# bcgsc/NanoSim

Measured on NVIDIA H100. Metric: simulated_bases_per_sec, higher is better.
Workload: dtype u8

## Files before the change

nanosim_b200/csrc/emit_kernel.cuh:

```cuda
#pragma once
#include "device_common.cuh"

#define EMIT_WARPS 8
#define EMIT_RING 256
#ifndef EMIT_MIN_BLOCKS
#define EMIT_MIN_BLOCKS 3
#endif

#ifndef EMIT_TMA_WINDOW
#define EMIT_TMA_WINDOW 1
#endif
#define EMIT_WIN_WORDS 64
#define EMIT_WINDOW_SMEM (EMIT_TMA_WINDOW ? EMIT_WARPS * (EMIT_WIN_WORDS * 4 + 8) : 0)

#define EMIT_F_RND 1u
#define EMIT_F_REF 4u
#define EMIT_F_MIS 8u

struct EmitArgs {
    DevRef ref;
    DevCfg cfg;
    uint32_t kind;
    uint32_t force_exact;
    uint64_t first_id;
    const NsReadMeta* reads;
    const NsPieceMeta* pieces;
    const uint32_t* ops;
    uint32_t n_pieces;
    uint8_t* seq;
    uint8_t* qual;
    const uint32_t* qlut;
    uint32_t* counter;
    const uint32_t* order;
    const uint32_t* abort;
    const uint32_t* split_base;
    const uint2* extra;
    const uint4* ckpt;
    const uint32_t* n_extra;
    uint32_t cap_extra;
};

#define EMIT_SPLIT 16384u

__device__ __forceinline__ uint32_t warp_incl_scan(uint32_t v, int lane) {
#pragma unroll
    for (int d = 1; d < 32; d <<= 1) {
        uint32_t t = __shfl_up_sync(0xffffffffu, v, d);
        if (lane >= d) v += t;
    }
    return v;
}

__device__ __forceinline__ uint32_t emit_op_info(uint32_t op, bool unmapped, bool ref_comp = false) {
    const uint32_t ty = op >> 28;
    const uint32_t qs = unmapped ? 4u : (ty == NS_OP_LIT ? ((op >> 24) & 3u) : ((0x30102u >> (4u * ty)) & 7u));
    uint32_t info = (qs * QLUT_SIZE * 4u) << 16;
    const uint32_t zero = ref_comp ? (uint32_t)'T' : (uint32_t)'A';
    if (ty < 2u) info |= EMIT_F_REF | (ty == NS_OP_MIS ? EMIT_F_MIS : 0u) | (zero << 8);
    else if (ty == NS_OP_LIT) info |= idx_base(((op >> 26) & 3u) ^ (ref_comp ? 2u : 0u)) << 8;
    else info |= 3u | (zero << 8);
    return info;
}

struct ChunkAux {
    uint32_t RB;
    uint32_t X[3];
};
template <bool FASTQ>
struct ChunkQual {
    uint32_t W[FASTQ ? 16 : 1];
    uint32_t X[4];
};

template <bool FASTQ>
__device__ __forceinline__ void draw_chunk_aux(ChunkAux& r, uint32_t id_lo, uint32_t id_hi, uint32_t kind, uint32_t chunk, uint2 key) {
    const uint4 a = FASTQ ? philox4x32_7(make_uint4(id_lo, id_hi, stream_word(ST_EMIT_Q, kind, chunk), 4u), key)
                          : philox4x32_7(make_uint4(id_lo, id_hi, stream_word(ST_EMIT_B, kind, chunk), 0u), key);
    r.RB = a.x; r.X[0] = a.y; r.X[1] = a.z; r.X[2] = a.w;
}
template <bool FASTQ>
__device__ __forceinline__ void draw_chunk_qual(ChunkQual<FASTQ>& r, uint32_t id_lo, uint32_t id_hi, uint32_t kind, uint32_t chunk, uint2 key) {
    if (FASTQ) {
        const uint32_t sw = stream_word(ST_EMIT_Q, kind, chunk);
#pragma unroll
        for (int j = 0; j < 4; ++j) {
            const uint4 t = philox4x32_7(make_uint4(id_lo, id_hi, sw, (uint32_t)j), key);
            r.W[4 * j] = t.x; r.W[4 * j + 1] = t.y; r.W[4 * j + 2] = t.z; r.W[4 * j + 3] = t.w;
            r.X[j] = __byte_perm(__byte_perm(t.x, t.y, 0x0040), __byte_perm(t.z, t.w, 0x0040), 0x5410);
        }
    } else {
        const uint4 b = philox4x32_7(make_uint4(id_lo, id_hi, stream_word(ST_EMIT_B, kind, chunk), 1u), key);
        r.X[0] = b.x; r.X[1] = b.y; r.X[2] = b.z; r.X[3] = b.w;
        r.W[0] = 0;
    }
}

__device__ __forceinline__ uint32_t sub_offsets(const uint32_t (&XA)[3], const uint32_t (&XB)[4]) {
    uint32_t sub = XA[0];
#pragma unroll
    for (int j = 1; j < 7; ++j) {
        const uint32_t z = ~(sub | (sub >> 1)) & 0x55555555u;
        sub |= (j < 3 ? XA[j] : XB[j - 3]) & (z * 3u);
    }
    return sub | (~(sub | (sub >> 1)) & 0x55555555u);
}
__device__ __forceinline__ uint32_t add_fields_mod4(uint32_t a, uint32_t b) {
    return a ^ b ^ ((a & b & 0x55555555u) << 1);
}

__device__ __forceinline__ uint32_t qual_pick(uint32_t e, uint32_t w) {
    return ((w | 0x7ffffu) < e) ? e : (e >> 8);
}

struct EmitPiece {
    const uint8_t* cbase;
    uint32_t pos, clen;
    uint32_t rdir;
    uint32_t ref_comp;
    uint32_t tbl;
    uint32_t piece_in_read;
    uint64_t rid;
};

__device__ __forceinline__ uint32_t entry_ref(const uint4& e, uint32_t rdir, uint32_t p) { return rdir ? e.y - p : e.y + p; }

__device__ __noinline__ uint32_t emit_fix_base(const EmitArgs& a, const EmitPiece& pc, const uint4* ring, uint32_t w_ret,
                                               uint32_t w_loaded, uint32_t x, uint32_t rb2, uint32_t misoff) {
    uint32_t l = w_ret, h = w_loaded;
    while (h - l > 1) {
        uint32_t mid = (l + h) >> 1;
        if (ring[mid & (EMIT_RING - 1)].x <= 2u * x) l = mid; else h = mid;
    }
    const uint4 e = ring[l & (EMIT_RING - 1)];
    const uint32_t info = e.w;
    uint32_t oi;
    if (info & EMIT_F_REF) {
        uint32_t rabs = entry_ref(e, pc.rdir, x);
        if (rabs >= pc.clen) rabs += pc.rdir ? pc.clen : 0u - pc.clen;
        uint32_t c = __ldg(pc.cbase + rabs);
        if (c - 'a' < 26u) c -= 32;
        if (!acgt_fast(c)) {
            const uint32_t f = rabs >= pc.pos ? rabs - pc.pos : rabs + pc.clen - pc.pos;
            c = converted_ref_base(c, a.cfg.seed, pc.rid, pc.piece_in_read, f);
        }
        oi = base_idx(c) ^ (pc.ref_comp ? 2u : 0u);
        if (info & EMIT_F_MIS) oi = (oi + misoff) & 3u;
    } else {
        oi = (info & 3u) ? rb2 : (base_idx((info >> 8) & 0xffu) ^ (pc.ref_comp ? 2u : 0u));
    }
    return (pc.tbl >> (8u * oi)) & 0xffu;
}

template <bool FASTQ, bool WRAPS, bool COMP>
__device__ __forceinline__ void emit_chunk16(const uint4* ring, const uint32_t* lut, const uint8_t* cvt_tables,
                                             const uint8_t* __restrict__ cbase, uint32_t RB, uint32_t sub, const ChunkQual<FASTQ>& Q,
                                             uint32_t& k, uint32_t& rem, uint32_t& rabs, uint32_t& info, uint32_t rdir, uint32_t clen,
                                             uint32_t wrap_fix, uint32_t tbl, uint32_t (&sb)[4], uint32_t (&sq)[4], uint32_t& bad) {
    const uint8_t* cvt = cvt_tables + (COMP ? 256 : 0);
    const uint32_t dir = rdir ? 0xffffffffu : 1u;
    uint32_t sel = 0;
#pragma unroll
    for (int i = 0; i < 16; ++i) {
        if (rem == 0) {
            ++k;
            const uint4 e = ring[k & (EMIT_RING - 1)];
            rem = (e.z - e.x) >> 1;
            rabs = entry_ref(e, rdir, e.x >> 1);
            info = e.w;
        }
        --rem;
        uint32_t c = (info >> 8) & 0xffu;
        if (info & EMIT_F_REF) {
            c = __ldg(cbase + rabs);
            rabs += dir;
            if (WRAPS && rabs >= clen) rabs += wrap_fix;
        }
        const uint32_t code = cvt[c];
        bad |= code;
        uint32_t v = code | ((RB >> (2 * i)) & info & 3u);
        if (info & EMIT_F_MIS) v += (sub >> (2 * i)) & 3u;
        sel += v << (4 * (i & 3));
        if (FASTQ) {
            const uint32_t w = Q.W[i];
            const uint32_t e = *reinterpret_cast<const uint32_t*>(reinterpret_cast<const char*>(lut) + (info >> 16) +
                                                                  ((w >> 6) & 0x1ffcu));
            sq[i >> 2] |= (qual_pick(e, w) & 0xffu) << (8 * (i & 3));
        }
        if ((i & 3) == 3) {
            sb[i >> 2] = __byte_perm(tbl, 0, sel & 0x3333u);
            sel = 0;
        }
    }
}

__device__ __forceinline__ uint32_t reverse_pairs(uint32_t x) {
    x = __brev(x);
    return ((x & 0x55555555u) << 1) | ((x >> 1) & 0x55555555u);
}
__device__ __forceinline__ uint32_t spread_pairs(uint32_t h) {
    uint32_t t = (h | (h << 8)) & 0x00ff00ffu;
    t = (t | (t << 4)) & 0x0f0f0f0fu;
    return (t | (t << 2)) & 0x33333333u;
}
__device__ __forceinline__ uint32_t bit_mask(uint32_t pos, uint32_t width) {
    uint32_t m;
    asm("bmsk.clamp.b32 %0, %1, %2;" : "=r"(m) : "r"(pos), "r"(width));
    return m;
}

__device__ __forceinline__ void load_packed_pair(const uint32_t* __restrict__ pk, uint32_t widx, uint32_t win_s, uint32_t win_w0,
                                                 uint32_t& w0, uint32_t& w1) {
#if EMIT_TMA_WINDOW
    const uint32_t rel = widx - win_w0;
    if (rel < EMIT_WIN_WORDS - 1u) {
        asm("ld.shared.u32 %0, [%2];\n\tld.shared.u32 %1, [%2+4];" : "=r"(w0), "=r"(w1) : "r"(win_s + 4u * rel));
        return;
    }
#endif
    w0 = __ldg(pk + widx);
    w1 = __ldg(pk + widx + 1);
}

template <bool RDIR>
__device__ __forceinline__ uint32_t emit_walk_entries(uint32_t ring_s, const uint32_t* __restrict__ pk, uint32_t pk0w, uint32_t win_s,
                                                      uint32_t win_w0, uint32_t RB, uint32_t& k, uint32_t cs, uint32_t& S, uint32_t& mism) {
    uint32_t acc = 0;
    S = 0xaaaaaaaau;
    mism = 0;
    const uint32_t cs2 = 2u * cs;
    for (;;) {
        uint4 e;
        asm("ld.shared.v4.u32 {%0, %1, %2, %3}, [%4];" : "=r"(e.x), "=r"(e.y), "=r"(e.z), "=r"(e.w) : "r"(ring_s + ((k & (EMIT_RING - 1)) << 4)));
        const uint32_t info = e.w;
        const int32_t d0 = (int32_t)(e.x - cs2);
        const uint32_t lo2 = (uint32_t)(d0 > 0 ? d0 : 0);
        const uint32_t d1 = e.z - cs2;
        const uint32_t hi2 = d1 < 32u ? d1 : 32u;
        const uint32_t m = bit_mask(lo2, hi2 - lo2);
        if (info & EMIT_F_REF) {
            const uint32_t p = cs + (lo2 >> 1);
            uint32_t r16;
            if (!RDIR) {
                const uint32_t l = e.y + p;
                uint32_t w0, w1;
                load_packed_pair(pk, pk0w + (l >> 4), win_s, win_w0, w0, w1);
                r16 = __funnelshift_r(w0, w1, (l + l) & 30u);
            } else {
                const uint32_t l1 = e.y - p + 1u;
                uint32_t w0, w1;
                load_packed_pair(pk, pk0w + (l1 >> 4) - 1u, win_s, win_w0, w0, w1);
                r16 = reverse_pairs(__funnelshift_r(w0, w1, (l1 + l1) & 30u));
            }
            acc = (acc & ~m) | ((r16 << lo2) & m);
            if (info & EMIT_F_MIS) mism |= m;
        } else {
            const uint32_t v = (info & EMIT_F_RND) ? RB : ((info >> 9) & 3u) * 0x55555555u;
            acc = (acc & ~m) | (v & m);
            S = (S & ~m) | (((info >> 29) * 0x55555555u) & m);
        }
        if (d1 >= 32u) break;
        ++k;
    }
    return acc;
}

template <bool FASTQ>
__device__ __forceinline__ void emit_chunk16_fast(uint32_t ring_s, const char* lut_s, const uint32_t* __restrict__ pk, uint32_t pk0w,
                                                  uint32_t win_s, uint32_t win_w0, uint32_t& k,
                                                  uint32_t cs, bool rdir, bool unmapped, uint32_t tbl, uint32_t id_lo, uint32_t id_hi,
                                                  uint32_t kind, uint32_t chunk, uint2 key, uint32_t (&sb)[4], uint32_t (&sq)[4]) {
    ChunkAux R;
    draw_chunk_aux<FASTQ>(R, id_lo, id_hi, kind, chunk, key);
    uint32_t S, mism;
    uint32_t acc = rdir ? emit_walk_entries<true>(ring_s, pk, pk0w, win_s, win_w0, R.RB, k, cs, S, mism)
                        : emit_walk_entries<false>(ring_s, pk, pk0w, win_s, win_w0, R.RB, k, cs, S, mism);
    ChunkQual<FASTQ> Q;
    draw_chunk_qual<FASTQ>(Q, id_lo, id_hi, kind, chunk, key);
    acc = add_fields_mod4(acc, sub_offsets(R.X, Q.X) & mism);
    S &= ~mism;
    {
        const uint32_t s0 = spread_pairs(acc & 0xffffu), s1 = spread_pairs(acc >> 16);
        sb[0] = __byte_perm(tbl, 0, s0);
        sb[1] = __byte_perm(tbl, 0, s0 >> 16);
        sb[2] = __byte_perm(tbl, 0, s1);
        sb[3] = __byte_perm(tbl, 0, s1 >> 16);
    }
    if (FASTQ) {
        if (unmapped) S = 0;
        uint32_t q[16];
#pragma unroll
        for (int i = 0; i < 16; ++i) {
            const uint32_t w = Q.W[i];
            const uint32_t st = (2 * i <= 13) ? (S << (13 - 2 * i)) : (S >> (2 * i - 13));
            const uint32_t off = (st & 0x6000u) | ((w >> 6) & 0x1ffcu);
            q[i] = qual_pick(*reinterpret_cast<const uint32_t*>(lut_s + off), w);
        }
#pragma unroll
        for (int g = 0; g < 4; ++g)
            sq[g] = __byte_perm(__byte_perm(q[4 * g], q[4 * g + 1], 0x0040), __byte_perm(q[4 * g + 2], q[4 * g + 3], 0x0040), 0x5410);
    }
}

template <bool FASTQ>
__global__ void __launch_bounds__(EMIT_WARPS * 32, EMIT_MIN_BLOCKS) emit_kernel(const __grid_constant__ EmitArgs a) {
    if (a.abort && *a.abort) return;
    extern __shared__ uint4 smem4[];
    uint32_t* lut = reinterpret_cast<uint32_t*>(smem4);
    uint8_t* cvt_tables = reinterpret_cast<uint8_t*>(lut + (FASTQ ? NS_N_QUAL_STATES * QLUT_SIZE : 0));
    const int lane = threadIdx.x & 31, warp = threadIdx.x >> 5;
    uint4* ring = reinterpret_cast<uint4*>(cvt_tables + 512) + warp * EMIT_RING;
    const uint32_t ring_s = (uint32_t)__cvta_generic_to_shared(ring);
#if EMIT_TMA_WINDOW
    const uint32_t win_s = (uint32_t)__cvta_generic_to_shared(reinterpret_cast<uint4*>(cvt_tables + 512) + EMIT_WARPS * EMIT_RING) +
                           warp * (EMIT_WIN_WORDS * 4);
    const uint32_t mbar_s = win_s + (EMIT_WARPS - warp) * (EMIT_WIN_WORDS * 4) + warp * 8;
    uint32_t win_phase = 0;
    if (lane == 0) {
        asm volatile("mbarrier.init.shared::cta.b64 [%0], 1;" ::"r"(mbar_s));
        asm volatile("fence.mbarrier_init.release.cluster;" ::: "memory");
    }
#else
    const uint32_t win_s = 0;
#endif
    if (FASTQ)
        for (int i = threadIdx.x; i < NS_N_QUAL_STATES * QLUT_SIZE; i += blockDim.x) lut[i] = a.qlut[i];
    {
        uint32_t c = threadIdx.x;
        uint32_t u = (c - 'a' < 26u) ? c - 32u : c;
        cvt_tables[c] = (uint8_t)(acgt_fast(u) ? base_idx(u) : 4u);
        cvt_tables[256 + c] = (uint8_t)(acgt_fast(u) ? base_idx(u) ^ 2u : 4u);
    }
    __syncthreads();
    const uint2 key = make_uint2((uint32_t)a.cfg.seed, (uint32_t)(a.cfg.seed >> 32));
    const uint32_t lane_lt = (1u << lane) - 1u;

    uint32_t n_extra = a.split_base ? *a.n_extra : 0u;
    if (n_extra > a.cap_extra) n_extra = a.cap_extra;
    for (;;) {
        uint32_t piece = 0, sub = 0;
        if (lane == 0) piece = atomicAdd(a.counter, 1u);
        piece = __shfl_sync(0xffffffffu, piece, 0);
        if (piece >= n_extra + a.n_pieces) break;
        if (piece < n_extra) {
            const uint2 x = a.extra[piece];
            if (x.x == 0xffffffffu) continue;
            piece = x.x;
            sub = x.y;
        } else {
            piece -= n_extra;
            if (a.order) piece = __ldg(&a.order[piece]);
        }
        const NsPieceMeta pm = a.pieces[piece];
        if (pm.out_len == 0) continue;
        const NsReadMeta rm = a.reads[pm.read_slot];
        const bool rev = rm.reversed != 0;
        const bool ref_comp = (pm.kind & NS_PIECE_REF_REV) != 0;
        const bool rdir = rev != ref_comp;
        const uint32_t n_ops = pm.n_ops, ref_len = pm.ref_len;
        const uint32_t A = rev ? rm.seq_len - pm.out_rel - pm.out_len : pm.out_rel;
        uint32_t pad = A & 15u;
        const uint32_t P0 = A - pad;
        uint32_t x_end = pad + pm.out_len;
        uint32_t t_first = 0, out_first = pad, ref_first = 0, x_first = 0;
        {
            const uint32_t sbase = a.split_base ? __ldg(&a.split_base[piece]) : 0xffffffffu;
            if (sbase != 0xffffffffu) {
                if (sub) {
                    const uint4 ck = a.ckpt[sbase + sub - 1u];
                    t_first = ck.x;
                    out_first = ck.y;
                    ref_first = ck.z;
                    x_first = sub * EMIT_SPLIT;
                    pad = 0;
                }
                if (x_end > (sub + 1u) * EMIT_SPLIT) x_end = (sub + 1u) * EMIT_SPLIT;
            }
        }
        const uint64_t cstart = a.ref.chrom_off[pm.chrom];
        EmitPiece pc;
        pc.cbase = a.ref.bases + cstart;
        pc.pos = pm.pos;
        pc.clen = (uint32_t)(a.ref.chrom_off[pm.chrom + 1] - cstart);
        pc.rdir = rdir;
        pc.ref_comp = ref_comp;
        {
            const uint32_t t = a.cfg.uracil ? 0x47554341u : 0x47544341u;
            pc.tbl = rev ? __byte_perm(t, 0, 0x1032) : t;
        }
        pc.piece_in_read = piece - rm.piece_first;
        pc.rid = a.first_id + pm.read_slot;
        const uint8_t* __restrict__ cbase = pc.cbase;
        const uint32_t clen = pc.clen, tbl = pc.tbl;
        const bool wraps = (uint64_t)pm.pos + ref_len > clen;
        const uint32_t wrap_fix = rdir ? clen : 0u - clen;
        const uint32_t* __restrict__ ops = a.ops + pm.op_off;
        uint8_t* seq_out = a.seq + rm.seq_off + P0;
        uint8_t* qual_out = FASTQ ? a.qual + rm.seq_off + P0 : nullptr;
        const bool unmapped = NS_PIECE_KIND(pm.kind) != NS_PIECE_SEGMENT;
        const uint32_t id_lo = (uint32_t)pc.rid, id_hi = (uint32_t)(pc.rid >> 32);
        const uint32_t info_pad = emit_op_info(NS_OP_HT << 28, unmapped, ref_comp);
        const uint64_t pk0 = a.ref.pk_off[pm.chrom];
        bool fast = !wraps && !ref_comp && !a.force_exact;
        if (fast && ref_len) {
            const uint64_t w_lo = pk0 + (pm.pos >> 4), w_hi = pk0 + ((pm.pos + ref_len - 1u) >> 4);
            fast = __ldg(&a.ref.exc_pre[(w_hi >> REF_EXC_BLOCK_SHIFT) + 1]) == __ldg(&a.ref.exc_pre[w_lo >> REF_EXC_BLOCK_SHIFT]);
        }
        const char* lut_s = reinterpret_cast<const char*>(lut) + (unmapped ? 4u * QLUT_SIZE * 4u : 0u);

        uint32_t t_loaded = t_first, w_loaded = 0, w_ret = 0, out_loaded = out_first, ref_loaded = ref_first, prog = x_first;
        bool closed = false;
        if (pad) {
            if (lane == 0) ring[0] = make_uint4(0u, 0u, 2u * pad, info_pad);
            w_loaded = 1;
        }
        auto put_entry = [&](uint32_t slot, uint32_t xo, uint32_t rstart, uint32_t len, uint32_t op) {
            uint32_t ab = pm.pos + (rdir ? ref_len - 1u - rstart : rstart);
            if (wraps && ab >= clen) ab -= clen;
            ring[slot & (EMIT_RING - 1)] = make_uint4(2u * xo, rdir ? ab + xo : ab - xo, 2u * (xo + len), emit_op_info(op, unmapped, ref_comp));
        };
        while (prog < x_end) {
            uint32_t target = prog + 512u < x_end ? prog + 512u : x_end;
            while (out_loaded < target && t_loaded < n_ops && (w_loaded - w_ret) + 65u <= EMIT_RING) {
                const uint32_t t = t_loaded + 2u * lane;
                uint32_t op0 = 0, op1 = 0;
                if (t < n_ops) op0 = __ldg(&ops[rev ? n_ops - 1u - t : t]);
                if (t + 1u < n_ops) op1 = __ldg(&ops[rev ? n_ops - 2u - t : t + 1u]);
                const uint32_t ty0 = op0 >> 28, len0 = op_len(op0), ty1 = op1 >> 28, len1 = op_len(op1);
                const uint32_t o0 = (ty0 == NS_OP_DEL) ? 0u : len0, o1 = (ty1 == NS_OP_DEL) ? 0u : len1;
                const uint32_t r0 = (ty0 < 2u || ty0 == NS_OP_DEL) ? len0 : 0u, r1 = (ty1 < 2u || ty1 == NS_OP_DEL) ? len1 : 0u;
                const uint32_t so = warp_incl_scan(o0 + o1, lane), sr = warp_incl_scan(r0 + r1, lane);
                const uint32_t bal0 = __ballot_sync(0xffffffffu, o0 != 0u), bal1 = __ballot_sync(0xffffffffu, o1 != 0u);
                const uint32_t slot = w_loaded + __popc(bal0 & lane_lt) + __popc(bal1 & lane_lt);
                const uint32_t xo = out_loaded + so - (o0 + o1), rs = ref_loaded + sr - (r0 + r1);
                if (o0) put_entry(slot, xo, rs, len0, op0);
                if (o1) put_entry(slot + (o0 ? 1u : 0u), xo + o0, rs + r0, len1, op1);
                out_loaded += __shfl_sync(0xffffffffu, so, 31);
                ref_loaded += __shfl_sync(0xffffffffu, sr, 31);
                w_loaded += __popc(bal0) + __popc(bal1);
                t_loaded += (n_ops - t_loaded < 64u) ? n_ops - t_loaded : 64u;
            }
            if (!closed && (t_loaded == n_ops || out_loaded >= x_end)) {
                if (lane == 0) ring[w_loaded & (EMIT_RING - 1)] = make_uint4(2u * out_loaded, 0u, 2u * out_loaded + 0x7ffffffeu, info_pad);
                ++w_loaded;
                closed = true;
            }
            __syncwarp();
            uint32_t win_w0 = (uint32_t)a.ref.pk_words + 4096u;
#if EMIT_TMA_WINDOW
            if (fast) {
                uint32_t kk = w_ret;
                uint4 e = ring[kk & (EMIT_RING - 1)];
                while (!(e.w & EMIT_F_REF) && kk + 1u < w_loaded) {
                    ++kk;
                    e = ring[kk & (EMIT_RING - 1)];
                }
                if (e.w & EMIT_F_REF) {
                    const uint32_t x0 = e.x >> 1;
                    const uint32_t w = (uint32_t)pk0 + (entry_ref(e, rdir, x0 > prog ? x0 : prog) >> 4);
                    win_w0 = !rdir ? (w & ~3u) : (w + 1u >= EMIT_WIN_WORDS - 1u ? (w + 1u - (EMIT_WIN_WORDS - 4u)) & ~3u : 0u);
                    if (lane == 0) {
                        asm volatile("mbarrier.arrive.expect_tx.shared::cta.b64 _, [%0], %1;" ::"r"(mbar_s), "r"(EMIT_WIN_WORDS * 4) : "memory");
                        asm volatile("cp.async.bulk.shared::cluster.global.mbarrier::complete_tx::bytes [%0], [%1], %2, [%3];"
                                     ::"r"(win_s), "l"(a.ref.packed + win_w0), "r"(EMIT_WIN_WORDS * 4), "r"(mbar_s) : "memory");
                    }
                }
            }
            const bool win_on = win_w0 < (uint32_t)a.ref.pk_words;
#endif
            uint32_t lim = out_loaded < target ? out_loaded : target;
            if (lim < x_end) lim &= ~15u;
            const uint32_t cs = prog + 16u * lane;
            uint32_t k = w_ret;
            if (cs < lim) {
                uint32_t l = w_ret, h = w_loaded;
                while (h - l > 1) {
                    uint32_t mid = (l + h) >> 1;
                    if (ring[mid & (EMIT_RING - 1)].x <= 2u * cs) l = mid; else h = mid;
                }
                k = l;
                const uint32_t chunk = (P0 + cs) >> 4;
                uint32_t sb[4], sq[4] = {0, 0, 0, 0};
                if (fast) {
#if EMIT_TMA_WINDOW
                    if (win_on) {
                        asm volatile("{\n\t.reg .pred p;\n\tWIN_WAIT:\n\tmbarrier.try_wait.parity.shared::cta.b64 p, [%0], %1;\n\t@p bra WIN_DONE;\n\tbra WIN_WAIT;\n\tWIN_DONE:\n\t}"
                                     ::"r"(mbar_s), "r"(win_phase) : "memory");
                    }
#endif
                    emit_chunk16_fast<FASTQ>(ring_s, lut_s, a.ref.packed, (uint32_t)pk0, win_s, win_w0, k, cs, rdir, unmapped, tbl, id_lo, id_hi, a.kind, chunk, key, sb, sq);
                } else {
                    ChunkAux R;
                    ChunkQual<FASTQ> Q;
                    draw_chunk_aux<FASTQ>(R, id_lo, id_hi, a.kind, chunk, key);
                    draw_chunk_qual<FASTQ>(Q, id_lo, id_hi, a.kind, chunk, key);
                    const uint32_t sub = sub_offsets(R.X, Q.X);
                    uint32_t rem, rabs, info;
                    {
                        const uint4 e = ring[k & (EMIT_RING - 1)];
                        rem = (e.z >> 1) - cs;
                        info = e.w;
                        rabs = entry_ref(e, rdir, cs);
                        if (wraps && rabs >= clen) rabs += wrap_fix;
                    }
                    uint32_t bad = 0;
                    if (ref_comp) emit_chunk16<FASTQ, true, true>(ring, lut, cvt_tables, cbase, R.RB, sub, Q, k, rem, rabs, info, rdir, clen, wrap_fix, tbl, sb, sq, bad);
                    else if (wraps) emit_chunk16<FASTQ, true, false>(ring, lut, cvt_tables, cbase, R.RB, sub, Q, k, rem, rabs, info, rdir, clen, wrap_fix, tbl, sb, sq, bad);
                    else emit_chunk16<FASTQ, false, false>(ring, lut, cvt_tables, cbase, R.RB, sub, Q, k, rem, rabs, info, rdir, clen, wrap_fix, tbl, sb, sq, bad);
                    if (bad & 4u) {
#pragma unroll
                        for (int i = 0; i < 16; ++i) {
                            const uint32_t f = emit_fix_base(a, pc, ring, w_ret, w_loaded, cs + i, (R.RB >> (2 * i)) & 3u, (sub >> (2 * i)) & 3u);
                            const uint32_t m = 0xffu << (8 * (i & 3));
                            sb[i >> 2] = (sb[i >> 2] & ~m) | (f << (8 * (i & 3)));
                        }
                    }
                }
                if (cs >= pad && cs + 16u <= x_end) {
                    *reinterpret_cast<uint4*>(seq_out + cs) = make_uint4(sb[0], sb[1], sb[2], sb[3]);
                    if (FASTQ) *reinterpret_cast<uint4*>(qual_out + cs) = make_uint4(sq[0], sq[1], sq[2], sq[3]);
                } else {
#pragma unroll
                    for (int i = 0; i < 16; ++i) {
                        if (cs + i >= pad && cs + i < x_end) {
                            seq_out[cs + i] = (uint8_t)(sb[i >> 2] >> (8 * (i & 3)));
                            if (FASTQ) qual_out[cs + i] = (uint8_t)(sq[i >> 2] >> (8 * (i & 3)));
                        }
                    }
                }
            }
            {
                const uint32_t n_act = (lim - prog + 15u) >> 4;
                const uint32_t k_last = __shfl_sync(0xffffffffu, k, n_act ? n_act - 1u : 0u);
                if (n_act) w_ret = k_last;
            }
            prog = lim;
            __syncwarp();
#if EMIT_TMA_WINDOW
            if (win_on) win_phase ^= 1u;
#endif
        }
    }
}

struct SplitArgs {
    const NsReadMeta* reads;
    const NsPieceMeta* pieces;
    const uint32_t* ops;
    uint32_t n_pieces;
    uint32_t* split_base;
    uint2* extra;
    uint4* ckpt;
    uint32_t* n_extra;
    uint32_t cap_extra;
    const uint32_t* abort;
};

__global__ void __launch_bounds__(256) split_kernel(const __grid_constant__ SplitArgs a) {
    if (a.abort && *a.abort) return;
    const int lane = threadIdx.x & 31;
    const uint32_t lane_lt = (1u << lane) - 1u;
    (void)lane_lt;
    const uint32_t n_warps = gridDim.x * (blockDim.x >> 5);
    for (uint32_t piece = blockIdx.x * (blockDim.x >> 5) + (threadIdx.x >> 5); piece < a.n_pieces; piece += n_warps) {
        const NsPieceMeta* pmp = a.pieces + piece;
        const uint32_t out_len = pmp->out_len;
        if (out_len <= EMIT_SPLIT - 16u) {
            if (lane == 0) a.split_base[piece] = 0xffffffffu;
            continue;
        }
        const NsPieceMeta pm = *pmp;
        const NsReadMeta rm = a.reads[pm.read_slot];
        const bool rev = rm.reversed != 0;
        const uint32_t A = rev ? rm.seq_len - pm.out_rel - pm.out_len : pm.out_rel;
        const uint32_t pad = A & 15u, x_end = pad + out_len;
        const uint32_t n_sub = (x_end + EMIT_SPLIT - 1u) / EMIT_SPLIT;
        if (n_sub < 2u) {
            if (lane == 0) a.split_base[piece] = 0xffffffffu;
            continue;
        }
        uint32_t base = 0;
// ... 46 lines not shown
```

nanosim_b200/csrc/nanosim_api.cu:

```cuda
#include <cuda_runtime.h>
#include <cub/device/device_radix_sort.cuh>
#include <cub/device/device_scan.cuh>

#include <algorithm>
#include <cstdarg>
#include <cstdio>
#include <cstring>
#include <dlfcn.h>
#include <string>
#include <memory>
#include <vector>

#if __has_include(<nccl.h>)
#include <nccl.h>
#define NS_HAVE_NCCL 1
#else
#define NS_HAVE_NCCL 0
#endif

#include "nanosim_b200.h"
#include "device_common.cuh"
#include "plan_kernel.cuh"
#include "emit_kernel.cuh"
#include "uread_kernel.cuh"
// ... 490 lines not shown

int launch_emit(NsContext* ctx, int kind, uint64_t first_read_id, uint32_t n_pieces, const uint32_t* order,
                const uint32_t* abort_flag = nullptr, bool split = true, cudaEvent_t emit_begin = nullptr) {
    cudaStream_t st = ctx->stream;
    EmitArgs ea;
    ea.ref = dev_ref(ctx);
    ea.cfg = ctx->dcfg;
    ea.kind = (uint32_t)kind;
    ea.first_id = first_read_id;
    ea.reads = ctx->reads.as<NsReadMeta>();
    ea.pieces = ctx->pieces.as<NsPieceMeta>();
    ea.ops = ctx->ops.as<uint32_t>();
    ea.n_pieces = n_pieces;
    ea.seq = ctx->seq.as<uint8_t>();
    ea.qual = ctx->qual.as<uint8_t>();
    ea.qlut = ctx->tables->qlut.as<uint32_t>();
    ea.force_exact = (ctx->hcfg.flags & NS_FLAG_EMIT_EXACT) ? 1u : 0u;
    ea.abort = abort_flag;
    ea.counter = ctx->counter.as<uint32_t>();
    ea.order = order;
    CK(cudaMemsetAsync(ctx->counter.p, 0, 64, st));
    {
        const uint32_t cap_extra = (uint32_t)std::min<size_t>(ctx->seq.cap / (EMIT_SPLIT - 16u) + 64u, 0x7fffffffu);
        ea.split_base = nullptr;
        ea.extra = nullptr;
        ea.ckpt = nullptr;
        ea.n_extra = ctx->counter.as<uint32_t>() + 4;
        ea.cap_extra = cap_extra;
        if (split && n_pieces && !(ctx->hcfg.flags & NS_FLAG_EMIT_WHOLE)) {
            CK(ctx->split_base.ensure((size_t)n_pieces * sizeof(uint32_t)));
            CK(ctx->split_extra.ensure((size_t)cap_extra * sizeof(uint2)));
            CK(ctx->split_ckpt.ensure((size_t)cap_extra * sizeof(uint4)));
            CK(cudaMemsetAsync(ctx->split_extra.p, 0xff, (size_t)cap_extra * sizeof(uint2), st));
            SplitArgs sa;
            sa.reads = ea.reads;
            sa.pieces = ea.pieces;
            sa.ops = ea.ops;
            sa.n_pieces = n_pieces;
            sa.split_base = ctx->split_base.as<uint32_t>();
            sa.extra = ctx->split_extra.as<uint2>();
            sa.ckpt = ctx->split_ckpt.as<uint4>();
            sa.n_extra = ctx->counter.as<uint32_t>() + 4;
            sa.cap_extra = cap_extra;
            sa.abort = abort_flag;
            const unsigned sblocks = std::min<unsigned>((n_pieces + 7u) / 8u, (unsigned)ctx->sm_count * 8u);
            CK(launch(ctx, split_kernel, sblocks, 256, 0, sa));
            if (emit_begin) CK(cudaEventRecord(emit_begin, st));
            ea.split_base = sa.split_base;
            ea.extra = sa.extra;
            ea.ckpt = sa.ckpt;
        }
    }
    void (*kernel)(EmitArgs) = ctx->hcfg.fastq ? emit_kernel<true> : emit_kernel<false>;
    const size_t smem = (size_t)EMIT_WARPS * EMIT_RING * sizeof(uint4) + 512 + EMIT_WINDOW_SMEM +
                        (ctx->hcfg.fastq ? (size_t)NS_N_QUAL_STATES * QLUT_SIZE * 4 : 0);
    CK(cudaFuncSetAttribute(kernel, cudaFuncAttributeMaxDynamicSharedMemorySize, (int)smem));
    int per_sm = 1;
    CK(cudaOccupancyMaxActiveBlocksPerMultiprocessor(&per_sm, kernel, EMIT_WARPS * 32, smem));
    const unsigned blocks = std::min<unsigned>((n_pieces + EMIT_WARPS - 1) / EMIT_WARPS, (unsigned)(ctx->sm_count * std::max(per_sm, 1)));
    CK(launch(ctx, kernel, blocks, EMIT_WARPS * 32, smem, ea));
    return NS_OK;
}

}

extern "C" {

int ns_create(int device, uint64_t seed, NsContext** out) {
    if (!out) return NS_EINVAL;
    *out = nullptr;
    NsContext* ctx = new NsContext();
    ctx->device = device;
    ctx->seed = seed;
    cudaError_t e = cudaSetDevice(device);
    if (e == cudaSuccess) e = cudaStreamCreateWithFlags(&ctx->stream, cudaStreamNonBlocking);
    for (int i = 0; i < 6 && e == cudaSuccess; ++i) e = cudaEventCreate(&ctx->ev[i].e);
    if (e == cudaSuccess) e = ctx->h_totals.ensure(16 * sizeof(uint64_t), cudaHostAllocMapped);
    if (e == cudaSuccess) e = cudaHostGetDevicePointer((void**)&ctx->h_totals_dev, ctx->h_totals.p, 0);
    if (e == cudaSuccess && device >= 0 && device < 64 && !g_base[device]) {
        e = cudaEventCreate(&g_base[device]);
        if (e == cudaSuccess) e = cudaEventRecord(g_base[device], ctx->stream);
        if (e == cudaSuccess) e = cudaEventSynchronize(g_base[device]);
    }
    if (e == cudaSuccess) {
        cudaDeviceProp prop;
        e = cudaGetDeviceProperties(&prop, device);
        if (e == cudaSuccess) ctx->sm_count = prop.multiProcessorCount;
    }
    if (e != cudaSuccess) {
        fprintf(stderr, "nanosim_b200: ns_create failed: %s\n", cudaGetErrorString(e));
        delete ctx;
        return NS_ECUDA;
    }
    *out = ctx;
    return NS_OK;
}

int ns_destroy(NsContext* ctx) {
    if (!ctx) return NS_EINVAL;
    cudaSetDevice(ctx->device);
    cudaStreamSynchronize(ctx->stream);
    delete ctx;
    return NS_OK;
}

const char* ns_last_error(const NsContext* ctx) { return ctx ? ctx->err.c_str() : "null context"; }

int ns_clone(NsContext* parent, NsContext** out) {
// ... 1190 lines not shown
```

Measured before the change: 120.2 billion.

## Compress emit ring entries to 8 bytes and double ring capacity

Ring entries shrink from uint4 (x-start, ref, x-end, info) to uint2, packing the output offset and op info into one word. An entry's end is now read from the next entry's start. Ring depth doubles to 512 in the same shared memory, and the reverse-complement conversion table is replaced by a bit trick. The exact path moves into a helper, and split pieces use piece-relative coordinates, which lowers shared-memory footprint and load width per entry at the cost of an extra neighbour load and a 24-bit limit on offsets.

```diff
diff --git a/nanosim_b200/csrc/emit_kernel.cuh b/nanosim_b200/csrc/emit_kernel.cuh
--- a/nanosim_b200/csrc/emit_kernel.cuh
+++ b/nanosim_b200/csrc/emit_kernel.cuh
@@ -2,7 +2,8 @@
 #include "device_common.cuh"
 
 #define EMIT_WARPS 8
-#define EMIT_RING 256
+#define EMIT_RING 512
+#define EMIT_STEP 512u
 #ifndef EMIT_MIN_BLOCKS
 #define EMIT_MIN_BLOCKS 3
 #endif
@@ -12,10 +13,12 @@
 #endif
 #define EMIT_WIN_WORDS 64
 #define EMIT_WINDOW_SMEM (EMIT_TMA_WINDOW ? EMIT_WARPS * (EMIT_WIN_WORDS * 4 + 8) : 0)
-
-#define EMIT_F_RND 1u
+#define EMIT_SMEM (256 + EMIT_WARPS * EMIT_RING * 8 + EMIT_WINDOW_SMEM)
+
 #define EMIT_F_REF 4u
 #define EMIT_F_MIS 8u
+#define EMIT_F_RND 16u
+#define EMIT_X_END 0xffffffu
 
 struct EmitArgs {
     DevRef ref;
@@ -51,16 +54,17 @@
     return v;
 }
 
-__device__ __forceinline__ uint32_t emit_op_info(uint32_t op, bool unmapped, bool ref_comp = false) {
+__device__ __forceinline__ uint32_t emit_op_info(uint32_t op, bool unmapped) {
+    static_assert(QLUT_SIZE * 4 == 1 << 13, "alias table of a quality state: 8 KB");
     const uint32_t ty = op >> 28;
     const uint32_t qs = unmapped ? 4u : (ty == NS_OP_LIT ? ((op >> 24) & 3u) : ((0x30102u >> (4u * ty)) & 7u));
-    uint32_t info = (qs * QLUT_SIZE * 4u) << 16;
-    const uint32_t zero = ref_comp ? (uint32_t)'T' : (uint32_t)'A';
-    if (ty < 2u) info |= EMIT_F_REF | (ty == NS_OP_MIS ? EMIT_F_MIS : 0u) | (zero << 8);
-    else if (ty == NS_OP_LIT) info |= idx_base(((op >> 26) & 3u) ^ (ref_comp ? 2u : 0u)) << 8;
-    else info |= 3u | (zero << 8);
+    uint32_t info = qs << 5;
+    if (ty < 2u) info |= EMIT_F_REF | (ty == NS_OP_MIS ? EMIT_F_MIS : 0u);
+    else if (ty == NS_OP_LIT) info |= (op >> 26) & 3u;
+    else info |= EMIT_F_RND;
     return info;
 }
+__device__ __forceinline__ uint32_t info_qual_off(uint32_t info) { return (info & 0xe0u) << 8; }
 
 struct ChunkAux {
     uint32_t RB;
@@ -122,17 +126,18 @@
     uint64_t rid;
 };
 
-__device__ __forceinline__ uint32_t entry_ref(const uint4& e, uint32_t rdir, uint32_t p) { return rdir ? e.y - p : e.y + p; }
-
-__device__ __noinline__ uint32_t emit_fix_base(const EmitArgs& a, const EmitPiece& pc, const uint4* ring, uint32_t w_ret,
+__device__ __forceinline__ uint32_t entry_x(uint32_t ex) { return ex >> 8; }
+__device__ __forceinline__ uint32_t entry_ref(const uint2& e, uint32_t rdir, uint32_t p) { return rdir ? e.y - p : e.y + p; }
+
+__device__ __noinline__ uint32_t emit_fix_base(const EmitArgs& a, const EmitPiece& pc, const uint2* ring, uint32_t w_ret,
                                                uint32_t w_loaded, uint32_t x, uint32_t rb2, uint32_t misoff) {
     uint32_t l = w_ret, h = w_loaded;
     while (h - l > 1) {
         uint32_t mid = (l + h) >> 1;
-        if (ring[mid & (EMIT_RING - 1)].x <= 2u * x) l = mid; else h = mid;
-    }
-    const uint4 e = ring[l & (EMIT_RING - 1)];
-    const uint32_t info = e.w;
+        if (entry_x(ring[mid & (EMIT_RING - 1)].x) <= x) l = mid; else h = mid;
+    }
+    const uint2 e = ring[l & (EMIT_RING - 1)];
+    const uint32_t info = e.x;
     uint32_t oi;
     if (info & EMIT_F_REF) {
         uint32_t rabs = entry_ref(e, pc.rdir, x);
@@ -146,43 +151,44 @@
         oi = base_idx(c) ^ (pc.ref_comp ? 2u : 0u);
         if (info & EMIT_F_MIS) oi = (oi + misoff) & 3u;
     } else {
-        oi = (info & 3u) ? rb2 : (base_idx((info >> 8) & 0xffu) ^ (pc.ref_comp ? 2u : 0u));
+        oi = (info & EMIT_F_RND) ? rb2 : (info & 3u);
     }
     return (pc.tbl >> (8u * oi)) & 0xffu;
 }
 
 template <bool FASTQ, bool WRAPS, bool COMP>
-__device__ __forceinline__ void emit_chunk16(const uint4* ring, const uint32_t* lut, const uint8_t* cvt_tables,
+__device__ __forceinline__ void emit_chunk16(const uint2* ring, const uint32_t* lut, const uint8_t* cvt,
                                              const uint8_t* __restrict__ cbase, uint32_t RB, uint32_t sub, const ChunkQual<FASTQ>& Q,
                                              uint32_t& k, uint32_t& rem, uint32_t& rabs, uint32_t& info, uint32_t rdir, uint32_t clen,
                                              uint32_t wrap_fix, uint32_t tbl, uint32_t (&sb)[4], uint32_t (&sq)[4], uint32_t& bad) {
-    const uint8_t* cvt = cvt_tables + (COMP ? 256 : 0);
     const uint32_t dir = rdir ? 0xffffffffu : 1u;
     uint32_t sel = 0;
 #pragma unroll
     for (int i = 0; i < 16; ++i) {
         if (rem == 0) {
             ++k;
-            const uint4 e = ring[k & (EMIT_RING - 1)];
-            rem = (e.z - e.x) >> 1;
-            rabs = entry_ref(e, rdir, e.x >> 1);
-            info = e.w;
+            const uint2 e = ring[k & (EMIT_RING - 1)];
+            const uint32_t x0 = entry_x(e.x);
+            rem = entry_x(ring[(k + 1u) & (EMIT_RING - 1)].x) - x0;
+            rabs = entry_ref(e, rdir, x0);
+            info = e.x;
         }
         --rem;
-        uint32_t c = (info >> 8) & 0xffu;
+        uint32_t code = info & 3u;
         if (info & EMIT_F_REF) {
-            c = __ldg(cbase + rabs);
+            const uint32_t c = __ldg(cbase + rabs);
             rabs += dir;
             if (WRAPS && rabs >= clen) rabs += wrap_fix;
-        }
-        const uint32_t code = cvt[c];
+            code = cvt[c];
+            if (COMP) code ^= (~code >> 1) & 2u;
+        }
         bad |= code;
-        uint32_t v = code | ((RB >> (2 * i)) & info & 3u);
+        uint32_t v = (info & EMIT_F_RND) ? (RB >> (2 * i)) & 3u : code;
         if (info & EMIT_F_MIS) v += (sub >> (2 * i)) & 3u;
         sel += v << (4 * (i & 3));
         if (FASTQ) {
             const uint32_t w = Q.W[i];
-            const uint32_t e = *reinterpret_cast<const uint32_t*>(reinterpret_cast<const char*>(lut) + (info >> 16) +
+            const uint32_t e = *reinterpret_cast<const uint32_t*>(reinterpret_cast<const char*>(lut) + info_qual_off(info) +
                                                                   ((w >> 6) & 0x1ffcu));
             sq[i >> 2] |= (qual_pick(e, w) & 0xffu) << (8 * (i & 3));
         }
@@ -221,21 +227,25 @@
     w1 = __ldg(pk + widx + 1);
 }
 
+__device__ __forceinline__ uint2 ring_ld(uint32_t ring_s, uint32_t k) {
+    uint2 e;
+    asm("ld.shared.v2.u32 {%0, %1}, [%2];" : "=r"(e.x), "=r"(e.y) : "r"(ring_s + ((k & (EMIT_RING - 1)) << 3)));
+    return e;
+}
+
 template <bool RDIR>
 __device__ __forceinline__ uint32_t emit_walk_entries(uint32_t ring_s, const uint32_t* __restrict__ pk, uint32_t pk0w, uint32_t win_s,
                                                       uint32_t win_w0, uint32_t RB, uint32_t& k, uint32_t cs, uint32_t& S, uint32_t& mism) {
     uint32_t acc = 0;
     S = 0xaaaaaaaau;
     mism = 0;
-    const uint32_t cs2 = 2u * cs;
+    uint2 e = ring_ld(ring_s, k), n = ring_ld(ring_s, k + 1u);
     for (;;) {
-        uint4 e;
-        asm("ld.shared.v4.u32 {%0, %1, %2, %3}, [%4];" : "=r"(e.x), "=r"(e.y), "=r"(e.z), "=r"(e.w) : "r"(ring_s + ((k & (EMIT_RING - 1)) << 4)));
-        const uint32_t info = e.w;
-        const int32_t d0 = (int32_t)(e.x - cs2);
-        const uint32_t lo2 = (uint32_t)(d0 > 0 ? d0 : 0);
-        const uint32_t d1 = e.z - cs2;
-        const uint32_t hi2 = d1 < 32u ? d1 : 32u;
+        const uint32_t info = e.x;
+        const int32_t d0 = (int32_t)(entry_x(e.x) - cs);
+        const uint32_t lo2 = d0 > 0 ? 2u * (uint32_t)d0 : 0u;
+        const uint32_t d1 = entry_x(n.x) - cs;
+        const uint32_t hi2 = d1 < 16u ? 2u * d1 : 32u;
         const uint32_t m = bit_mask(lo2, hi2 - lo2);
         if (info & EMIT_F_REF) {
             const uint32_t p = cs + (lo2 >> 1);
@@ -254,12 +264,14 @@
             acc = (acc & ~m) | ((r16 << lo2) & m);
             if (info & EMIT_F_MIS) mism |= m;
         } else {
-            const uint32_t v = (info & EMIT_F_RND) ? RB : ((info >> 9) & 3u) * 0x55555555u;
+            const uint32_t v = (info & EMIT_F_RND) ? RB : (info & 3u) * 0x55555555u;
             acc = (acc & ~m) | (v & m);
-            S = (S & ~m) | (((info >> 29) * 0x55555555u) & m);
-        }
-        if (d1 >= 32u) break;
+            S = (S & ~m) | ((((info >> 5) & 3u) * 0x55555555u) & m);
+        }
+        if (d1 >= 16u) break;
         ++k;
+        e = n;
+        n = ring_ld(ring_s, k + 1u);
     }
     return acc;
 }
@@ -302,17 +314,70 @@
 }
 
 template <bool FASTQ>
+__device__ __forceinline__ void store_chunk(const EmitArgs& a, uint64_t out_off, uint32_t cs, uint32_t pad, uint32_t x_end,
+                                            const uint32_t (&sb)[4], const uint32_t (&sq)[4]) {
+    if (cs >= pad && cs + 16u <= x_end) {
+        *reinterpret_cast<uint4*>(a.seq + out_off + cs) = make_uint4(sb[0], sb[1], sb[2], sb[3]);
+        if (FASTQ) *reinterpret_cast<uint4*>(a.qual + out_off + cs) = make_uint4(sq[0], sq[1], sq[2], sq[3]);
+    } else {
+#pragma unroll
+        for (int i = 0; i < 16; ++i) {
+            if (cs + i >= pad && cs + i < x_end) {
+                a.seq[out_off + cs + i] = (uint8_t)(sb[i >> 2] >> (8 * (i & 3)));
+                if (FASTQ) a.qual[out_off + cs + i] = (uint8_t)(sq[i >> 2] >> (8 * (i & 3)));
+            }
+        }
+    }
+}
+
+template <bool FASTQ>
+__device__ __forceinline__ uint32_t emit_chunk_exact(const EmitArgs& a, const EmitPiece& pc, const uint2* ring, const uint32_t* lut,
+                                                  const uint8_t* cvt, uint32_t w_ret, uint32_t w_loaded, uint32_t k, uint32_t cs,
+                                                  uint32_t chunk, bool wraps, uint64_t out_off, uint32_t pad, uint32_t x_end) {
+    const uint2 key = make_uint2((uint32_t)a.cfg.seed, (uint32_t)(a.cfg.seed >> 32));
+    const uint32_t id_lo = (uint32_t)pc.rid, id_hi = (uint32_t)(pc.rid >> 32);
+    const uint32_t rdir = pc.rdir, clen = pc.clen, wrap_fix = rdir ? clen : 0u - clen;
+    ChunkAux R;
+    ChunkQual<FASTQ> Q;
+    draw_chunk_aux<FASTQ>(R, id_lo, id_hi, a.kind, chunk, key);
+    draw_chunk_qual<FASTQ>(Q, id_lo, id_hi, a.kind, chunk, key);
+    const uint32_t sub = sub_offsets(R.X, Q.X);
+    uint32_t rem, rabs, info;
+    {
+        const uint2 e = ring[k & (EMIT_RING - 1)];
+        rem = entry_x(ring[(k + 1u) & (EMIT_RING - 1)].x) - cs;
+        info = e.x;
+        rabs = entry_ref(e, rdir, cs);
+        if (wraps && rabs >= clen) rabs += wrap_fix;
+    }
+    uint32_t sb[4], sq[4] = {0, 0, 0, 0}, bad = 0;
+    if (pc.ref_comp) emit_chunk16<FASTQ, true, true>(ring, lut, cvt, pc.cbase, R.RB, sub, Q, k, rem, rabs, info, rdir, clen, wrap_fix, pc.tbl, sb, sq, bad);
+    else if (wraps) emit_chunk16<FASTQ, true, false>(ring, lut, cvt, pc.cbase, R.RB, sub, Q, k, rem, rabs, info, rdir, clen, wrap_fix, pc.tbl, sb, sq, bad);
+    else emit_chunk16<FASTQ, false, false>(ring, lut, cvt, pc.cbase, R.RB, sub, Q, k, rem, rabs, info, rdir, clen, wrap_fix, pc.tbl, sb, sq, bad);
+    if (bad & 4u) {
+#pragma unroll
+        for (int i = 0; i < 16; ++i) {
+            const uint32_t f = emit_fix_base(a, pc, ring, w_ret, w_loaded, cs + i, (R.RB >> (2 * i)) & 3u, (sub >> (2 * i)) & 3u);
+            const uint32_t m = 0xffu << (8 * (i & 3));
+            sb[i >> 2] = (sb[i >> 2] & ~m) | (f << (8 * (i & 3)));
+        }
+    }
+    store_chunk<FASTQ>(a, out_off, cs, pad, x_end, sb, sq);
+    return k;
+}
+
+template <bool FASTQ>
 __global__ void __launch_bounds__(EMIT_WARPS * 32, EMIT_MIN_BLOCKS) emit_kernel(const __grid_constant__ EmitArgs a) {
     if (a.abort && *a.abort) return;
     extern __shared__ uint4 smem4[];
     uint32_t* lut = reinterpret_cast<uint32_t*>(smem4);
-    uint8_t* cvt_tables = reinterpret_cast<uint8_t*>(lut + (FASTQ ? NS_N_QUAL_STATES * QLUT_SIZE : 0));
+    uint8_t* cvt = reinterpret_cast<uint8_t*>(lut + (FASTQ ? NS_N_QUAL_STATES * QLUT_SIZE : 0));
     const int lane = threadIdx.x & 31, warp = threadIdx.x >> 5;
-    uint4* ring = reinterpret_cast<uint4*>(cvt_tables + 512) + warp * EMIT_RING;
+    uint8_t* const rings = cvt + 256;
+    uint2* ring = reinterpret_cast<uint2*>(rings) + warp * EMIT_RING;
     const uint32_t ring_s = (uint32_t)__cvta_generic_to_shared(ring);
 #if EMIT_TMA_WINDOW
-    const uint32_t win_s = (uint32_t)__cvta_generic_to_shared(reinterpret_cast<uint4*>(cvt_tables + 512) + EMIT_WARPS * EMIT_RING) +
-                           warp * (EMIT_WIN_WORDS * 4);
+    const uint32_t win_s = (uint32_t)__cvta_generic_to_shared(rings + EMIT_WARPS * EMIT_RING * 8) + warp * (EMIT_WIN_WORDS * 4);
     const uint32_t mbar_s = win_s + (EMIT_WARPS - warp) * (EMIT_WIN_WORDS * 4) + warp * 8;
     uint32_t win_phase = 0;
     if (lane == 0) {
@@ -327,8 +392,7 @@
     {
         uint32_t c = threadIdx.x;
         uint32_t u = (c - 'a' < 26u) ? c - 32u : c;
-        cvt_tables[c] = (uint8_t)(acgt_fast(u) ? base_idx(u) : 4u);
-        cvt_tables[256 + c] = (uint8_t)(acgt_fast(u) ? base_idx(u) ^ 2u : 4u);
+        cvt[c] = (uint8_t)(acgt_fast(u) ? base_idx(u) : 4u);
     }
     __syncthreads();
     const uint2 key = make_uint2((uint32_t)a.cfg.seed, (uint32_t)(a.cfg.seed >> 32));
@@ -359,21 +423,23 @@
         const uint32_t n_ops = pm.n_ops, ref_len = pm.ref_len;
         const uint32_t A = rev ? rm.seq_len - pm.out_rel - pm.out_len : pm.out_rel;
         uint32_t pad = A & 15u;
-        const uint32_t P0 = A - pad;
+        uint32_t P0 = A - pad;
         uint32_t x_end = pad + pm.out_len;
-        uint32_t t_first = 0, out_first = pad, ref_first = 0, x_first = 0;
+        uint32_t t_first = 0, out_first = pad, ref_first = 0;
         {
             const uint32_t sbase = a.split_base ? __ldg(&a.split_base[piece]) : 0xffffffffu;
             if (sbase != 0xffffffffu) {
+                if (x_end > (sub + 1u) * EMIT_SPLIT) x_end = (sub + 1u) * EMIT_SPLIT;
                 if (sub) {
                     const uint4 ck = a.ckpt[sbase + sub - 1u];
+                    const uint32_t x_first = sub * EMIT_SPLIT;
                     t_first = ck.x;
-                    out_first = ck.y;
+                    out_first = ck.y - x_first;
                     ref_first = ck.z;
-                    x_first = sub * EMIT_SPLIT;
+                    P0 += x_first;
+                    x_end -= x_first;
                     pad = 0;
                 }
-                if (x_end > (sub + 1u) * EMIT_SPLIT) x_end = (sub + 1u) * EMIT_SPLIT;
             }
         }
         const uint64_t cstart = a.ref.chrom_off[pm.chrom];
@@ -389,16 +455,13 @@
         }
         pc.piece_in_read = piece - rm.piece_first;
         pc.rid = a.first_id + pm.read_slot;
-        const uint8_t* __restrict__ cbase = pc.cbase;
         const uint32_t clen = pc.clen, tbl = pc.tbl;
         const bool wraps = (uint64_t)pm.pos + ref_len > clen;
-        const uint32_t wrap_fix = rdir ? clen : 0u - clen;
         const uint32_t* __restrict__ ops = a.ops + pm.op_off;
-        uint8_t* seq_out = a.seq + rm.seq_off + P0;
-        uint8_t* qual_out = FASTQ ? a.qual + rm.seq_off + P0 : nullptr;
+        const uint64_t out_off = rm.seq_off + P0;
         const bool unmapped = NS_PIECE_KIND(pm.kind) != NS_PIECE_SEGMENT;
         const uint32_t id_lo = (uint32_t)pc.rid, id_hi = (uint32_t)(pc.rid >> 32);
-        const uint32_t info_pad = emit_op_info(NS_OP_HT << 28, unmapped, ref_comp);
+        const uint32_t info_pad = emit_op_info(NS_OP_HT << 28, unmapped);
         const uint64_t pk0 = a.ref.pk_off[pm.chrom];
         bool fast = !wraps && !ref_comp && !a.force_exact;
         if (fast && ref_len) {
@@ -407,20 +470,24 @@
         }
         const char* lut_s = reinterpret_cast<const char*>(lut) + (unmapped ? 4u * QLUT_SIZE * 4u : 0u);
 
-        uint32_t t_loaded = t_first, w_loaded = 0, w_ret = 0, out_loaded = out_first, ref_loaded = ref_first, prog = x_first;
+        uint32_t t_loaded = t_first, w_loaded = 0, w_ret = 0, out_loaded = out_first, ref_loaded = ref_first, prog = 0;
         bool closed = false;
         if (pad) {
-            if (lane == 0) ring[0] = make_uint4(0u, 0u, 2u * pad, info_pad);
+            if (lane == 0) ring[0] = make_uint2(info_pad, 0u);
             w_loaded = 1;
         }
+        auto entry_word = [&](uint32_t xo, uint32_t info) {
+            return ((uint32_t)min(max((int32_t)xo, 0), (int32_t)((x_end + 15u) & ~15u)) << 8) | info;
+        };
         auto put_entry = [&](uint32_t slot, uint32_t xo, uint32_t rstart, uint32_t len, uint32_t op) {
             uint32_t ab = pm.pos + (rdir ? ref_len - 1u - rstart : rstart);
             if (wraps && ab >= clen) ab -= clen;
-            ring[slot & (EMIT_RING - 1)] = make_uint4(2u * xo, rdir ? ab + xo : ab - xo, 2u * (xo + len), emit_op_info(op, unmapped, ref_comp));
+            const uint32_t ex = entry_word(xo, emit_op_info(op, unmapped));
+            ring[slot & (EMIT_RING - 1)] = make_uint2(ex, rdir ? ab + xo : ab - xo);
         };
         while (prog < x_end) {
-            uint32_t target = prog + 512u < x_end ? prog + 512u : x_end;
-            while (out_loaded < target && t_loaded < n_ops && (w_loaded - w_ret) + 65u <= EMIT_RING) {
+            const uint32_t target = prog + EMIT_STEP < x_end ? prog + EMIT_STEP : x_end;
+            while ((int32_t)out_loaded < (int32_t)target && t_loaded < n_ops && (w_loaded - w_ret) + 66u <= EMIT_RING) {
                 const uint32_t t = t_loaded + 2u * lane;
                 uint32_t op0 = 0, op1 = 0;
                 if (t < n_ops) op0 = __ldg(&ops[rev ? n_ops - 1u - t : t]);
@@ -439,26 +506,33 @@
                 w_loaded += __popc(bal0) + __popc(bal1);
                 t_loaded += (n_ops - t_loaded < 64u) ? n_ops - t_loaded : 64u;
             }
-            if (!closed && (t_loaded == n_ops || out_loaded >= x_end)) {
-                if (lane == 0) ring[w_loaded & (EMIT_RING - 1)] = make_uint4(2u * out_loaded, 0u, 2u * out_loaded + 0x7ffffffeu, info_pad);
+            if (!closed && (t_loaded == n_ops || (int32_t)out_loaded >= (int32_t)x_end)) {
+                if (lane == 0) {
+                    ring[w_loaded & (EMIT_RING - 1)] = make_uint2(entry_word(out_loaded, info_pad), 0u);
+                    ring[(w_loaded + 1u) & (EMIT_RING - 1)] = make_uint2((EMIT_X_END << 8) | info_pad, 0u);
+                }
                 ++w_loaded;
                 closed = true;
+            } else if (!closed && lane == 0) {
+                ring[w_loaded & (EMIT_RING - 1)].x = entry_word(out_loaded, 0u);
             }
             __syncwarp();
             uint32_t win_w0 = (uint32_t)a.ref.pk_words + 4096u;
 #if EMIT_TMA_WINDOW
             if (fast) {
                 uint32_t kk = w_ret;
-                uint4 e = ring[kk & (EMIT_RING - 1)];
-                while (!(e.w & EMIT_F_REF) && kk + 1u < w_loaded) {
+                if (entry_x(ring[(kk + 1u) & (EMIT_RING - 1)].x) <= prog) ++kk;
+                uint2 e = ring[kk & (EMIT_RING - 1)];
+                while (!(e.x & EMIT_F_REF) && kk + 1u < w_loaded) {
                     ++kk;
                     e = ring[kk & (EMIT_RING - 1)];
                 }
-                if (e.w & EMIT_F_REF) {
-                    const uint32_t x0 = e.x >> 1;
+                if (e.x & EMIT_F_REF) {
+                    const uint32_t x0 = entry_x(e.x);
                     const uint32_t w = (uint32_t)pk0 + (entry_ref(e, rdir, x0 > prog ? x0 : prog) >> 4);
                     win_w0 = !rdir ? (w & ~3u) : (w + 1u >= EMIT_WIN_WORDS - 1u ? (w + 1u - (EMIT_WIN_WORDS - 4u)) & ~3u : 0u);
-                    if (lane == 0) {
+                    if (win_w0 + EMIT_WIN_WORDS > (uint32_t)a.ref.pk_words) win_w0 = (uint32_t)a.ref.pk_words + 4096u;
+                    else if (lane == 0) {
                         asm volatile("mbarrier.arrive.expect_tx.shared::cta.b64 _, [%0], %1;" ::"r"(mbar_s), "r"(EMIT_WIN_WORDS * 4) : "memory");
                         asm volatile("cp.async.bulk.shared::cluster.global.mbarrier::complete_tx::bytes [%0], [%1], %2, [%3];"
                                      ::"r"(win_s), "l"(a.ref.packed + win_w0), "r"(EMIT_WIN_WORDS * 4), "r"(mbar_s) : "memory");
@@ -467,7 +541,7 @@
             }
             const bool win_on = win_w0 < (uint32_t)a.ref.pk_words;
 #endif
-            uint32_t lim = out_loaded < target ? out_loaded : target;
+            uint32_t lim = (int32_t)out_loaded < (int32_t)target ? out_loaded : target;
             if (lim < x_end) lim &= ~15u;
             const uint32_t cs = prog + 16u * lane;
             uint32_t k = w_ret;
@@ -475,11 +549,10 @@
                 uint32_t l = w_ret, h = w_loaded;
                 while (h - l > 1) {
                     uint32_t mid = (l + h) >> 1;
-                    if (ring[mid & (EMIT_RING - 1)].x <= 2u * cs) l = mid; else h = mid;
+                    if (entry_x(ring[mid & (EMIT_RING - 1)].x) <= cs) l = mid; else h = mid;
                 }
                 k = l;
                 const uint32_t chunk = (P0 + cs) >> 4;
-                uint32_t sb[4], sq[4] = {0, 0, 0, 0};
                 if (fast) {
 #if EMIT_TMA_WINDOW
                     if (win_on) {
@@ -487,45 +560,11 @@
                                      ::"r"(mbar_s), "r"(win_phase) : "memory");
                     }
 #endif
+                    uint32_t sb[4], sq[4] = {0, 0, 0, 0};
                     emit_chunk16_fast<FASTQ>(ring_s, lut_s, a.ref.packed, (uint32_t)pk0, win_s, win_w0, k, cs, rdir, unmapped, tbl, id_lo, id_hi, a.kind, chunk, key, sb, sq);
+                    store_chunk<FASTQ>(a, out_off, cs, pad, x_end, sb, sq);
                 } else {
-                    ChunkAux R;
-                    ChunkQual<FASTQ> Q;
-                    draw_chunk_aux<FASTQ>(R, id_lo, id_hi, a.kind, chunk, key);
-                    draw_chunk_qual<FASTQ>(Q, id_lo, id_hi, a.kind, chunk, key);
-                    const uint32_t sub = sub_offsets(R.X, Q.X);
-                    uint32_t rem, rabs, info;
-                    {
-                        const uint4 e = ring[k & (EMIT_RING - 1)];
-                        rem = (e.z >> 1) - cs;
-                        info = e.w;
-                        rabs = entry_ref(e, rdir, cs);
-                        if (wraps && rabs >= clen) rabs += wrap_fix;
-                    }
-                    uint32_t bad = 0;
-                    if (ref_comp) emit_chunk16<FASTQ, true, true>(ring, lut, cvt_tables, cbase, R.RB, sub, Q, k, rem, rabs, info, rdir, clen, wrap_fix, tbl, sb, sq, bad);
-                    else if (wraps) emit_chunk16<FASTQ, true, false>(ring, lut, cvt_tables, cbase, R.RB, sub, Q, k, rem, rabs, info, rdir, clen, wrap_fix, tbl, sb, sq, bad);
-                    else emit_chunk16<FASTQ, false, false>(ring, lut, cvt_tables, cbase, R.RB, sub, Q, k, rem, rabs, info, rdir, clen, wrap_fix, tbl, sb, sq, bad);
-                    if (bad & 4u) {
-#pragma unroll
-                        for (int i = 0; i < 16; ++i) {
-                            const uint32_t f = emit_fix_base(a, pc, ring, w_ret, w_loaded, cs + i, (R.RB >> (2 * i)) & 3u, (sub >> (2 * i)) & 3u);
-                            const uint32_t m = 0xffu << (8 * (i & 3));
-                            sb[i >> 2] = (sb[i >> 2] & ~m) | (f << (8 * (i & 3)));
-                        }
-                    }
-                }
-                if (cs >= pad && cs + 16u <= x_end) {
-                    *reinterpret_cast<uint4*>(seq_out + cs) = make_uint4(sb[0], sb[1], sb[2], sb[3]);
-                    if (FASTQ) *reinterpret_cast<uint4*>(qual_out + cs) = make_uint4(sq[0], sq[1], sq[2], sq[3]);
-                } else {
-#pragma unroll
-                    for (int i = 0; i < 16; ++i) {
-                        if (cs + i >= pad && cs + i < x_end) {
-                            seq_out[cs + i] = (uint8_t)(sb[i >> 2] >> (8 * (i & 3)));
-                            if (FASTQ) qual_out[cs + i] = (uint8_t)(sq[i >> 2] >> (8 * (i & 3)));
-                        }
-                    }
+                    k = emit_chunk_exact<FASTQ>(a, pc, ring, lut, cvt, w_ret, w_loaded, k, cs, chunk, wraps, out_off, pad, x_end);
                 }
             }
             {
diff --git a/nanosim_b200/csrc/nanosim_api.cu b/nanosim_b200/csrc/nanosim_api.cu
--- a/nanosim_b200/csrc/nanosim_api.cu
+++ b/nanosim_b200/csrc/nanosim_api.cu
@@ -566,8 +566,7 @@
         }
     }
     void (*kernel)(EmitArgs) = ctx->hcfg.fastq ? emit_kernel<true> : emit_kernel<false>;
-    const size_t smem = (size_t)EMIT_WARPS * EMIT_RING * sizeof(uint4) + 512 + EMIT_WINDOW_SMEM +
-                        (ctx->hcfg.fastq ? (size_t)NS_N_QUAL_STATES * QLUT_SIZE * 4 : 0);
+    const size_t smem = (size_t)EMIT_SMEM + (ctx->hcfg.fastq ? (size_t)NS_N_QUAL_STATES * QLUT_SIZE * 4 : 0);
     CK(cudaFuncSetAttribute(kernel, cudaFuncAttributeMaxDynamicSharedMemorySize, (int)smem));
     int per_sm = 1;
     CK(cudaOccupancyMaxActiveBlocksPerMultiprocessor(&per_sm, kernel, EMIT_WARPS * 32, smem));
```

Result: faster. 123.2 billion, median of 6 (+2.5%).
